# statsleelab/gauss

Measured on AMD Instinct MI355X. Metric: imputed SNPs/sec (whole node) at 1/2/4/8 GPUs; LD-GEMM MFMA TFLOP/s vs peak, higher is better.
Workload: dtype f32

## Files before the change

### gauss_amd/csrc/gauss_job.h

```cpp
#pragma once
#include "gauss_internal.h"
#pragma GCC visibility push(default)
#include "../../include/gauss_hip.h"
#pragma GCC visibility pop

#include <algorithm>
#include <atomic>
#include <chrono>
#include <condition_variable>
#include <cmath>
#include <cstdarg>
#include <cstdio>
#include <cstring>
#include <deque>
#include <functional>
#include <map>
#include <memory>
#include <mutex>
#include <set>
#include <shared_mutex>
#include <thread>
#include <string>
#include <vector>

// ... 258 lines not shown
    char* h_pin = nullptr;
    hipEvent_t begin = nullptr;
    hipEvent_t zeroed = nullptr;
    hipEvent_t done = nullptr;
    struct RunEvents { hipEvent_t gram = nullptr, side = nullptr, pack = nullptr, rows = nullptr, epi = nullptr; };
    RunEvents rev[2];
    Prob* d_probs = nullptr;
    Item* d_items = nullptr;    int n_items = 0;
    int2* d_rowmap = nullptr;   int n_rows = 0;
    std::unique_ptr<Plan> gplan;
    std::vector<int> g0;
    std::vector<std::vector<int2>> win_tiles;
    int2* d_tilemap = nullptr;  int n_tiles = 0;
    int n_tiles_b11 = 0;
    int n_items_b11 = 0;
    bool chain_aside = false;
    int2* d_panelmap = nullptr; int n_panels = 0;
    int2* d_dpanelmap = nullptr; int n_dpanels = 0;
    int2* d_gemmmap = nullptr;  int n_gemm = 0;
    int gemm_ut = 128;
    int2* d_finmap = nullptr;   int n_fin = 0;
    int* d_slctmap = nullptr;   int n_slct = 0;
    int* d_condmap = nullptr;   int n_cond = 0;
    int cond_max_U = 0;
    int* d_csmap = nullptr;     int n_cs = 0;
    int* d_prsmap = nullptr;    int n_prs = 0;
    int prs_max_s = 0, prs_max_M = 0;
    int cs_max_T = 0;
    int* d_susiemap = nullptr;  int n_susie = 0;
    int susie_max_M = 0, susie_max_U = 0, susie_max_T = 0;
    int susie_max_L = 0, susie_max_sweeps = 0, susie_max_nblk = 0;
    int susie_max_k = 0;  bool susie_coloc = false;
    int* d_xsmap = nullptr;     int n_xs = 0;
    int* d_xsleadmap = nullptr; int n_xs_lead = 0;
    int xs_max_M = 0, xs_max_U = 0, xs_max_T = 0, xs_max_L = 0, xs_max_sweeps = 0, xs_max_nblk = 0;
    int2* d_traitsmap = nullptr;  int n_traits = 0;
    int2* d_traitsumap = nullptr; int n_traits_u = 0;
    int2* d_missmap = nullptr;  int n_miss_blk = 0;
    int2* d_misstmap = nullptr; int n_miss_t = 0;
    int2* d_missumap = nullptr; int n_miss_u = 0;
    int2* d_loomap = nullptr;   int n_loo = 0;
    bool needs_fused() const
    { return std::any_of(plans.begin(), plans.end(), [](const Plan& pl) { return pl.rd.needs_fused(); }); }
    int max_nblk = 0;
    int max_npanel = 0;
    int solve_split = 0;
    int own_panel = 0;
    struct StreamGroup { int item0, n_items, row0, n_rows, tile0, n_tiles; };
    std::vector<StreamGroup> sgroups;
    std::vector<hipEvent_t> sevp;
    int max_pop = 1;
    int gram_i8 = 0;
    int gram_packed = 0;
    unsigned long long* d_code3 = nullptr;
    unsigned long long pack_stamp = 0;
    int resample_lds = -1;
    int* d_status = nullptr;
    unsigned long long* d_b11_done = nullptr;
    bool merged = false;
    bool force_merged = false;
    bool queue_touched = false;
    hipStream_t zero_queue = nullptr;
    double wait_bound_us = 0.0;
    unsigned long long merged_runs = 0;
    int n_items_b21_early = 0;
    int n_tiles_b21_early = 0;
    double* d_results = nullptr; size_t n_results = 0;
    double* h_res2[2] = {nullptr, nullptr};
    int* h_st2[2] = {nullptr, nullptr};
    hipEvent_t done2[2] = {nullptr, nullptr};
    unsigned run_seq = 0, fetch_seq = 0;
    double* h_results = nullptr;
    int* h_status = nullptr;
    struct Export { int plan, which; size_t off; int rows, width, pitch; double* user; };
    std::vector<Export> exports;
    std::vector<std::pair<int, int>> exp_chunks;
    std::vector<hipEvent_t> exp_ev;
    double* h_export = nullptr;
    ExportD* d_exports = nullptr;
    bool prof = false;
    std::vector<ProfSlot> slots;
    double prof_ms[5] = {0, 0, 0, 0, 0};
    long long prof_n[5] = {0, 0, 0, 0, 0};
    bool ran = false;
    bool ran_solve = true;
    unsigned prof_run = 0;
    long long n_merged = 0, n_demoted = 0, n_giveups = 0, n_rerun_failed = 0;
};

struct StreamSetup {
    uint8_t* d_m = nullptr;
    uint8_t* d_u = nullptr;
    long long ldraw = 0;
    size_t row_bytes = 0;
    int M = 0, U = 0;
    std::vector<int> first_tile;
    std::vector<int> tile_group;
    std::vector<hipEvent_t> ev;
    std::mutex mu;
    std::condition_variable cv;
    int recorded = 0, rc = 0;
    std::string err;
    int n_groups() const { return (int)first_tile.size() - 1; }
};

struct WinSpec {
// ... 61 lines not shown
```

### gauss_amd/csrc/gauss_plan.cpp

```cpp
#include "gauss_job.h"

static int seg_max_for(const std::vector<WinSpec>& specs)
{
    if (specs.size() >= 4) return 4096;
    double pairs = 0, kp = 0;
    for (const WinSpec& w : specs) {
        if (w.gene_off || w.pair_i || w.M < 1 || w.n_pop < 1 || w.n_pop > 64 || !w.pop_off) return SEG_MAX;
        int nc = 0;
        for (int c = 0; c < 3; c++) nc += (w.u_codings >> c) & 1;
        const double mt = (w.M + TILE - 1) / TILE, ut = ((double)w.U * std::max(nc, 1) + TILE - 1) / TILE;
        pairs += mt * (mt + 1) / 2 + ut * mt;
        kp = std::max(kp, w.draw_pop ? (double)w.n_drawn + 32.0 : (double)w.pop_off[w.n_pop] + 32.0 * w.n_pop);
    }
    const double want = pairs * kp / 1300.0;
    return (int)std::min<double>(SEG_MAX, std::max<double>(384.0, std::floor(want / KC) * KC));
}
static int group_target_for(size_t n_windows)
{
    return n_windows >= 4 ? 2048 : 0;
}
int plan_problem(const WinSpec& w, Plan& pl, int seg_max, int group_target)
{
    if (w.mode != GAUSS_MODE_POOLED && w.mode != GAUSS_MODE_WEIGHTED) return fail(GAUSS_E_INVALID, "bad mode %d", w.mode);
    if (w.n_pop < 1 || w.n_pop > 64) return fail(GAUSS_E_INVALID, "n_pop must be in 1..64 (got %d)", w.n_pop);
    if (!w.pop_off) return fail(GAUSS_E_INVALID, "pop_off is NULL");
    if (w.M < 1) return fail(GAUSS_E_INVALID, "need at least one measured SNP row (got %d)", w.M);
    if (w.U < 0) return fail(GAUSS_E_INVALID, "negative n_unmeasured");
    if (w.mode == GAUSS_MODE_WEIGHTED && !w.pop_wgt) return fail(GAUSS_E_INVALID, "pop_wgt is NULL in weighted mode");
    if (!w.geno_m || (w.U > 0 && !w.geno_u)) return fail(GAUSS_E_INVALID, "genotype pointer is NULL");
    for (int p = 0; p < w.n_pop; p++)
        if (w.pop_off[p + 1] < w.pop_off[p]) return fail(GAUSS_E_INVALID, "pop_off must be non-decreasing");
    if (w.pop_off[0] != 0) return fail(GAUSS_E_INVALID, "pop_off[0] must be 0");
    const int N = w.pop_off[w.n_pop];
    if (N < 1) return fail(GAUSS_E_INVALID, "no samples");
    if ((long long)N * 225 >= (1LL << 31)) return fail(GAUSS_E_RANGE, "%d samples exceed the exact-integer range (9.5 M)", N);
    if (w.geno_fmt != GAUSS_GENO_U8 && w.geno_fmt != GAUSS_GENO_2BIT) return fail(GAUSS_E_INVALID, "bad geno_format %d", w.geno_fmt);
    if (w.geno_fmt == GAUSS_GENO_U8 && w.ld < N) return fail(GAUSS_E_INVALID, "ld (%lld) < n_samples (%d)", w.ld, N);
    if (w.geno_fmt == GAUSS_GENO_2BIT) {
        if (w.ld % 16) return fail(GAUSS_E_INVALID, "2-bit rows need a stride that is a multiple of 16 bytes (got %lld)", w.ld);
        long long end = 0;
        for (int q = 0; q < w.n_pop; q++) {
            const long long blk = (long long)rup((size_t)(w.pop_off[q + 1] - w.pop_off[q]), 64) / 4;
            const long long off = w.pop_src_off ? w.pop_src_off[q] : end;
            if (off < 0 || off % 16) return fail(GAUSS_E_INVALID, "pop_src_off[%d] = %lld is not a multiple of 16", q, off);
            if (off + blk > w.ld) return fail(GAUSS_E_INVALID, "population block %d ends past the row stride", q);
            if (!w.pop_src_off) end = off + blk;
        }
    }
    if (w.kind != GAUSS_WIN_IMPUTE && w.kind != GAUSS_WIN_QCAT && w.kind != GAUSS_WIN_LD)
        return fail(GAUSS_E_INVALID, "bad window kind %d", w.kind);
    if (!w.ld_only && w.kind != GAUSS_WIN_LD && (w.U > 0 || w.kind == GAUSS_WIN_QCAT) && !w.z1) return fail(GAUSS_E_INVALID, "z1 is NULL");
    if (w.u_codings & ~(GAUSS_CODE_ADDITIVE | GAUSS_CODE_DOMINANT | GAUSS_CODE_RECESSIVE))
        return fail(GAUSS_E_INVALID, "bad u_codings mask %d", w.u_codings);
// ... 425 lines not shown
        for (int k = 0; k < K; k++) {
            const int i = mem[(size_t)k];
            const WinSpec& w = specs[(size_t)i];
            Plan::Riders& rd = plans[(size_t)i].rd;
            Prob& p = plans[(size_t)i].p;
            const char* differs = w.susie_L != a.susie_L ? "susie_L" : w.susie_coverage != a.susie_coverage ? "susie_coverage" :
                w.susie_prior_var != a.susie_prior_var ? "susie_prior_var" : w.susie_tol != a.susie_tol ? "susie_tol" :
                w.susie_min_abs_corr != a.susie_min_abs_corr ? "susie_min_abs_corr" : w.susie_max_sweeps != a.susie_max_sweeps ? "susie_max_sweeps" :
                (w.susie_estimate_var != 0) != (a.susie_estimate_var != 0) ? "susie_estimate_var" :
                (w.susie_measured_only != 0) != (a.susie_measured_only != 0) ? "susie_measured_only" : nullptr;
            if (differs) return fail(GAUSS_E_INVALID, "window %d: %s differs from the leader's (window %d): the windows of xs_group = %d share their susie_* arguments", i, differs, lead, id);
            const RiderOuts& o = w.out;
            if (k > 0 && (o.susie_pip || o.susie_set || o.susie_set_pip || o.susie_V || o.susie_lse || o.susie_mass || o.susie_purity || o.susie_size ||
                          o.susie_kept || o.susie_alpha || o.susie_mu || o.susie_sweeps || o.susie_lbf))
                return fail(GAUSS_E_INVALID, "window %d: out_susie_* on a peer of xs_group = %d: the joint fit is returned on the leader (window %d)", i, id, lead);
            if (k > 0 && (o.xs_V || o.xs_purity || o.xs_mu || o.xs_n))
                return fail(GAUSS_E_INVALID, "window %d: out_xs_* on a peer of xs_group = %d: they are the leader's (window %d)", i, id, lead);
            const int T = w.M + w.U;
            if (k > 0 && !w.xs_from_lead && (w.M != a.M || w.U != a.U))
                return fail(GAUSS_E_INVALID, "window %d: xs_from_lead is NULL (the same index) but n_measured / n_unmeasured = %d / %d differ from the leader's %d / %d",
                            i, w.M, w.U, a.M, a.U);
            if (w.xs_from_lead) {
                rd.xs_from_lead.assign(w.xs_from_lead, w.xs_from_lead + TL);
                rd.xs_to_lead.assign((size_t)T, -1);
                for (int j = 0; j < TL; j++) {
                    const int c = rd.xs_from_lead[(size_t)j];
                    if (c < -1 || c >= T)
                        return fail(GAUSS_E_INVALID, "window %d: xs_from_lead[%d] = %d is neither -1 nor a candidate of the window (0 .. %d)", i, j, c, T - 1);
                    if (c >= 0 && rd.xs_to_lead[(size_t)c] >= 0)
                        return fail(GAUSS_E_INVALID, "window %d: xs_from_lead[%d] = xs_from_lead[%d] = %d: two leader candidates cannot be one SNP", i,
                                    rd.xs_to_lead[(size_t)c], j, c);
                    if (c >= 0) rd.xs_to_lead[(size_t)c] = j;
                }
            }
            rd.xs_K = K; rd.xs_pos = k; rd.xs_lead = lead; rd.xs_mu = k == 0 && o.xs_mu != nullptr;
            p.xs_n = K; p.xs_pos = k; p.xs_mu = rd.xs_mu ? 1 : 0;
            for (int s = 0; s < XS_MAX; s++) p.xs_peer[s] = mem[(size_t)std::min(s, K - 1)];
        }
    }
    return GAUSS_OK;
}

int job_build(gauss_ctx* ctx, const std::vector<WinSpec>& specs, int on_device, gauss_job** out, const StreamSetup* stream)
{
    const bool streamed = stream != nullptr;
    const auto tb0 = std::chrono::steady_clock::now();
    gauss_job* job = new gauss_job();
    std::unique_ptr<gauss_job, void (*)(gauss_job*)> guard(job, job_free);
    job->ctx = ctx;
    job->n = (int)specs.size();
    job->on_device = on_device;
    job->gram_i8 = ctx->gram_i8;
    job->gram_packed = (ctx->gram_packed && !ctx->gram_i8) ? 1 : 0;
    job->plans.resize(job->n);
    for (const WinSpec& w : specs)
        if (w.draw_pop && (specs.size() != 1 || streamed)) return fail(GAUSS_E_INVALID, "a resampled window is a job of its own");
    const int seg_max = seg_max_for(specs);
    for (int i = 0; i < job->n; i++) {
        int rc = plan_problem(specs[i], job->plans[i], seg_max, group_target_for(specs.size()));
        if (rc) return rc;
        job->plans[i].p.gram_i8 = job->gram_i8;
        if (!job->plans[i].draw_col.empty()) job->resample_lds = resample_pack_lds_bytes(job->plans[i].p.row_src_bytes);
    }
    {
        const int rc = plan_xs_groups(specs, job->plans);
        if (rc) return rc;
    }
    size_t exp_doubles = 0;
    if (!streamed) {
        for (int i = 0; i < job->n; i++) {
            const Plan& pl = job->plans[i];
            const Prob& p = pl.p;
            const bool has = p.kind == GAUSS_WIN_LD || p.npanel > 0;
            if (!has) continue;
            if (pl.out_b11) { job->exports.push_back(gauss_job::Export{i, 0, exp_doubles, p.M, p.M, p.Mld, pl.out_b11}); exp_doubles += (size_t)p.M * p.M; }
            if (pl.out_b21 && p.U > 0) { job->exports.push_back(gauss_job::Export{i, 1, exp_doubles, p.U, p.M, p.Mld, pl.out_b21}); exp_doubles += (size_t)p.U * p.M; }
            exp_doubles = rup(exp_doubles, 32);
        }
        if (exp_doubles * sizeof(double) > ((size_t)256 << 20)) { job->exports.clear(); exp_doubles = 0; }
    }
    const auto tb1 = std::chrono::steady_clock::now();
    if (on_device && !streamed && job->n >= 2 && env_int("GAUSS_SHARE_MEASURED", 1) != 0) {
        const Plan& a = job->plans[0];
        bool ok = true;
        std::vector<int32_t> gl;
        std::vector<int> g0((size_t)job->n, 0);
        std::set<std::pair<int, int>> have;
        size_t cl0 = 0, own_pairs = 0;
        for (int i = 0; i < job->n && ok; i++) {
            const Plan& b = job->plans[i];
            ok = !b.rows_m.empty() && !b.p.ld_only && !b.p.n_gene && b.p.P <= 32 && b.h_geno_m == a.h_geno_m && b.user_ld == a.user_ld &&
                 b.p.mode == a.p.mode && b.p.P == a.p.P && b.p.geno_fmt == a.p.geno_fmt && b.p.slab16 == a.p.slab16 && b.p.Kp == a.p.Kp &&
                 b.pop_raw_off == a.pop_raw_off && b.pop_pk_off == a.pop_pk_off && b.pop_w == a.pop_w && b.seg_k0 == a.seg_k0 &&
                 b.seg_k1 == a.seg_k1 && b.seg_pop == a.seg_pop && b.run_src == a.run_src && b.run_pk_off == a.run_pk_off &&
                 b.groups == a.groups;
            if (!ok) break;
            const size_t M = b.rows_m.size(), mt = (M + TILE - 1) / TILE;
            own_pairs += mt * (mt + 1) / 2;
            size_t pos = gl.size();
            bool join = false;
            if (gl.size() > cl0 && std::is_sorted(gl.begin() + (ptrdiff_t)cl0, gl.end())) {
                const int32_t first = b.rows_m[0];
                const size_t p0 = (size_t)(std::lower_bound(gl.begin() + (ptrdiff_t)cl0, gl.end(), first) - gl.begin());
                if (p0 < gl.size() && gl[p0] == first) {
                    join = true;
                    for (size_t k = 0; k < M && join; k++) {
// ... 174 lines not shown
            for (int pr = 0; pr < p.npair; pr++) {
                const bool b21 = !p.ld_only && job->plans[i].pair_ti[pr] >= p.Mp / TILE;
                if (shm && !b21) continue;
                (b21 ? tilemap_b21 : tilemap).push_back(make_int2(i, pr));
                job->win_tiles[(size_t)i].push_back(make_int2(i, pr));
            }
        for (int pn = 0; pn < p.npi; pn++) panelmap.push_back(make_int2(i, pn));
        for (int pn = 0; pn < p.npanel; pn++) dpanelmap.push_back(make_int2(i, pn));
        const Plan::Riders& rd = job->plans[i].rd;
        if (rd.loo)
            for (int pn = 0; pn < (p.M + NR - 1) / NR; pn++) loomap.push_back(make_int2(i, pn));
        if (rd.slct_K) slctmap.push_back(i);
        if (rd.cond) { condmap.push_back(i); job->cond_max_U = std::max(job->cond_max_U, p.U); }
        if (rd.cs) { csmap.push_back(i); job->cs_max_T = std::max(job->cs_max_T, p.M + p.U); }
        if (rd.prs_n_s) { prsmap.push_back(i); job->prs_max_s = std::max(job->prs_max_s, rd.prs_n_s); job->prs_max_M = std::max(job->prs_max_M, p.M); }
        if (rd.susie_L && rd.xs_group) {
            xsmap.push_back(i);
            if (rd.xs_pos == 0) xsleadmap.push_back(i);
            job->xs_max_M = std::max(job->xs_max_M, p.M); job->xs_max_T = std::max(job->xs_max_T, p.M + p.U);
            job->xs_max_L = std::max(job->xs_max_L, rd.susie_L); job->xs_max_sweeps = std::max(job->xs_max_sweeps, p.susie_max_sweeps);
            if (!p.susie_measured_only) { job->xs_max_U = std::max(job->xs_max_U, p.U); job->xs_max_nblk = std::max(job->xs_max_nblk, p.nblk); }
        } else if (rd.susie_L) {
            susiemap.push_back(i);
            job->susie_max_M = std::max(job->susie_max_M, p.M); job->susie_max_T = std::max(job->susie_max_T, p.M + p.U);
            job->susie_max_L = std::max(job->susie_max_L, rd.susie_L); job->susie_max_sweeps = std::max(job->susie_max_sweeps, p.susie_max_sweeps);
            job->susie_max_k = std::max(job->susie_max_k, rd.susie_k); job->susie_coloc = job->susie_coloc || rd.coloc;
            if (!p.susie_measured_only) { job->susie_max_U = std::max(job->susie_max_U, p.U); job->susie_max_nblk = std::max(job->susie_max_nblk, p.nblk); }
        }
        if (rd.traits_T) {
            for (int b = 0; b < p.nblk; b++) traitsmap.push_back(make_int2(i, b));
            for (int us = 0; us < (p.U + NB - 1) / NB; us++) traitsumap.push_back(make_int2(i, us));
        }
        if (rd.miss) {
            if (p.miss_nm) for (int b = 0; b < p.nblk; b++) missmap.push_back(make_int2(i, b));
            for (int k = 0; k < p.miss_nm; k++) misstmap.push_back(make_int2(i, k));
            for (int us = 0; us < (p.U + NB - 1) / NB; us++) missumap.push_back(make_int2(i, us));
        }
        if (p.npanel > 0) {
            job->max_nblk = std::max(job->max_nblk, p.nblk); job->max_npanel = std::max(job->max_npanel, p.npi);
            for (int up = 0; up < p.Up128 / job->gemm_ut; up++)
                for (int kb = 0; kb < (p.Mld + 127) / 128; kb++) gemmmap.push_back(make_int2(i, (up << 8) | kb));
            for (int c = 0; c < (p.n_rhs + 255) / 256; c++) finmap.push_back(make_int2(i, c));
        }
        if (p.mode != 0) job->max_pop = std::max(job->max_pop, p.P);
    }
    {
        auto live_rows = [&](const Plan& pl, int t) {
            const Prob& p = pl.p;
            const int mt = p.Mp / TILE;
            if (!pl.tile_live.empty()) return pl.tile_live[(size_t)t];
            const int left = (t < mt) ? p.M - t * TILE : p.U - (t - mt) * TILE;
            return left > TILE ? TILE : left;
        };
        auto halves = [](int r, int w) { const int n = (r - w * 64 + 31) / 32; return n < 0 ? 0 : (n > 2 ? 2 : n); };
        for (ItemH& h : items) {
            h.ord = h.len;
            if (job->gram_i8) continue;
            const Plan& pl = plan_of(h.prob);
            const int ra = live_rows(pl, pl.pair_ti[h.pair]), rb = live_rows(pl, pl.pair_tj[h.pair]);
            const bool packed = job->gram_packed && pl.p.slab16;
            int mx = 0;
            for (int wr = 0; wr < 2; wr++)
                for (int wc = 0; wc < 2; wc++) mx = std::max(mx, (packed ? std::min(halves(ra, wr), 1) : halves(ra, wr)) * halves(rb, wc));
            h.ord = std::max(KC, (h.len * std::max(mx, 1) / 4 + KC - 1) / KC * KC);
        }
    }
    auto is_b11 = [&](const ItemH& h) { return h.b11 != 0; };
    std::vector<uint8_t> item_class(items.size(), 0);
    auto order_items = [&]() {
        int L = 0;
        bool whole = true;
        for (const ItemH& h : items) { L = std::max(L, h.ord / KC); whole = whole && h.ord % KC == 0 && h.ord >= 0; }
        if (!whole || (size_t)L > 4 * items.size() + 1024) {
            std::vector<size_t> idx(items.size());
            for (size_t n = 0; n < idx.size(); n++) idx[n] = n;
            std::stable_sort(idx.begin(), idx.end(), [&](size_t a, size_t b) {
                return item_class[a] != item_class[b] ? item_class[a] < item_class[b] : items[a].ord > items[b].ord; });
            std::vector<ItemH> out(items.size());
            for (size_t n = 0; n < idx.size(); n++) out[n] = items[idx[n]];
            items.swap(out);
            return;
        }
        const size_t nb = (size_t)3 * (size_t)(L + 1);
        std::vector<uint32_t> start(nb + 1, 0u);
        auto bucket = [&](size_t n) { return (size_t)item_class[n] * (size_t)(L + 1) + (size_t)(L - items[n].ord / KC); };
        for (size_t n = 0; n < items.size(); n++) start[bucket(n) + 1]++;
        for (size_t b = 0; b < nb; b++) start[b + 1] += start[b];
        std::vector<ItemH> out(items.size());
        for (size_t n = 0; n < items.size(); n++) out[start[bucket(n)]++] = items[n];
        items.swap(out);
    };
    {
        const int mode = env_int("GAUSS_CHAIN_ASIDE", 1);
        bool genes = false;
        double b21_len = 0.0;
        auto cost_len = [&](const ItemH& h) { return (double)h.len * ((job->gram_packed && plan_of(h.prob).p.slab16) ? GRAM_PACKED_COST : 1.0); };
        for (const ItemH& h : items) if (!is_b11(h)) b21_len += cost_len(h);
        for (int i = 0; i < job->n; i++) genes = genes || job->plans[i].p.n_gene > 0;
        const double t_b21 = b21_len * 2.0 * TILE * TILE / (job->gram_i8 ? 960e12 : 120e12), t_chain = 0.5e-3 + 100e-6 * job->max_nblk;
        {
            double all_len = 0.0;
            for (const ItemH& h : items) all_len += cost_len(h);
            job->wait_bound_us = 50.0 * 1e6 * all_len * 2.0 * TILE * TILE / (job->gram_i8 ? 960e12 : 120e12);
        }
        job->chain_aside = !streamed && mode != 0 && !panelmap.empty() && !tilemap_b21.empty() && !genes && job->ctx->chain &&
                           job->ctx->side && (mode == 2 || t_b21 >= 1.2 * t_chain);
        if (job->chain_aside)
            for (size_t n = 0; n < items.size(); n++) {
                item_class[n] = is_b11(items[n]) ? 0 : 1;
                job->n_items_b11 += is_b11(items[n]) ? 1 : 0;
            }
        {
            const int mm = env_int("GAUSS_CHAIN_MERGED", 1);
            job->merged = job->chain_aside && mm != 0 && (!job->gram_i8 || mm == 2);
            job->force_merged = job->merged && mm == 2;
        }
// ... 384 lines not shown
                return GAUSS_OK;
            };
            int rc = upload(w.raw_m, pl.h_geno_m, pl.rows_m, p.M);
            if (!rc) rc = upload(w.raw_u, pl.h_geno_u, pl.rows_u, pl.U_user);
            if (rc) return rc;
        }
    }
    if (shm) {
        Plan& g = *job->gplan;
        Prob& q = g.p;
        const size_t n = (size_t)job->n;
        char* T = job->d_tab;
        char* W = job->d_ws;
        q.ld_raw = g.user_ld;
        q.raw_m = g.h_geno_m; q.raw_u = nullptr;
        q.packed = (uint8_t*)(W + go.packed); q.packed_u = q.packed;
        q.sx = (int*)(W + go.sx); q.sxx = (int*)(W + go.sxx); q.sx_u = q.sx; q.sxx_u = q.sxx;
        q.rt_sd = (double*)(W + go.sd); q.rt_wm = (double*)(W + go.wm); q.rt_sd_u = q.rt_sd; q.rt_wm_u = q.rt_wm;
        q.rt_mu = (double*)(W + go.mu); q.rt_wmu = (double*)(W + go.wmu); q.rt_mu_u = q.rt_mu; q.rt_wmu_u = q.rt_wmu;
        q.pop_raw_off = (const int*)(T + to[n].raw_off); q.pop_pk_off = (const int*)(T + to[n].pk_off);
        q.pop_w = (const double*)(T + to[n].w); q.pop_wf = (const double*)(T + to[n].wf); q.pop_md = (const double*)(T + to[n].md);
        q.seg_pop = (const int*)(T + to[n].seg_pop); q.seg_k0 = (const int*)(T + to[n].k0); q.seg_k1 = (const int*)(T + to[n].k1);
        q.pop_seg0 = (const int*)(T + to[n].seg0);
        q.pair_ti = (const int*)(T + to[n].ti); q.pair_tj = (const int*)(T + to[n].tj); q.pair_lut = (const int*)(T + to[n].lut);
        q.word_pop = (const uint8_t*)(T + to[n].wp); q.word_run = (const uint8_t*)(T + to[n].wr);
        q.rows_m = (const int*)(T + to[n].rm); q.rows_u = nullptr;
        q.run_pk_off = (const int*)(T + to[n].rpk); q.run_src = (const int*)(T + to[n].rsrc);
        q.slab = (float*)(W + go.slab); q.slab_g = q.slab; q.gpair_ti = q.pair_ti; q.gpair_tj = q.pair_tj; q.g0 = 0; q.n_gpair = q.npair;
        q.z1 = nullptr; q.A = nullptr; q.B21 = nullptr; q.Linv = nullptr; q.V = nullptr; q.Gsum = nullptr; q.Part = nullptr;
        q.out_z = q.out_info = nullptr; clear_riders(q); q.out_ld = nullptr; q.status = job->d_status;
        q.gene_off = nullptr; q.gene_out_off = nullptr; q.n_gene = 0;
        memcpy(blob.data() + o_probs + sizeof(Prob) * n, &q, sizeof(Prob));
    }
    for (size_t n = 0; n < items.size(); n++) {
        const ItemH& h = items[n];
        const Plan& pl = plan_of(h.prob);
        const Prob& p = pl.p;
        const std::pair<int, int>& gr = h.group >= 0 ? pl.groups[h.group] : pl.fine[(size_t)(-1 - h.group)];
        const int ti = pl.pair_ti[h.pair], tj = pl.pair_tj[h.pair];
        const int mt = p.Mp / TILE;
        auto rows = [&](int t) {
            if (!pl.tile_live.empty()) return pl.tile_live[(size_t)t];
            int left = (t < mt) ? p.M - t * TILE : p.U - (t - mt) * TILE; return left > TILE ? TILE : left;
        };
        auto tile_rows = [&](int t) { return t < mt ? p.packed + (size_t)t * TILE * p.Kp : p.packed_u + (size_t)(t - mt) * TILE * p.Kp; };
        Item it;
        it.a = tile_rows(ti);
        it.b = tile_rows(tj);
        it.slab = p.slab + ((size_t)h.pair * p.nseg + gr.first) * (p.slab16 ? TILE * TILE / 2 : TILE * TILE);
        it.seg_k1 = p.seg_k1 + gr.first;
        it.chunk_live = (const uint32_t*)(job->d_tab + to[h.prob].ch);
        it.Kp = p.Kp; it.k0 = pl.seg_k0[gr.first]; it.nseg = gr.second - gr.first;
        it.rows_a = rows(ti); it.rows_b = rows(tj); it.flags = (ti == tj ? 1 : 0) | (p.slab16 ? 2 : 0) | (p.slab16 && job->gram_packed ? 4 : 0);
        if (job->merged && (int)n < job->n_items_b11) it.flags |= 16;
        else if (job->merged && (int)n < job->n_items_b11 + job->n_items_b21_early) it.flags |= 32;
        memcpy(blob.data() + o_items + sizeof(Item) * n, &it, sizeof(Item));
    }
    for (size_t x = 0; x < job->exports.size(); x++) {
        const gauss_job::Export& ex = job->exports[x];
        const Plan& pl = job->plans[(size_t)ex.plan];
        ExportD d;
        d.src = ex.which ? pl.p.B21 : (pl.p.kind == GAUSS_WIN_LD ? pl.p.A : pl.d_b11_copy);
        d.dst = job->h_export + ex.off;
        d.rows = ex.rows; d.width = ex.width; d.pitch = ex.pitch; d.pad_ = 0;
        memcpy(blob.data() + o_exports + sizeof(ExportD) * x, &d, sizeof(ExportD));
    }
    const auto tj2 = std::chrono::steady_clock::now();
    memcpy(job->h_pin, blob.data(), blob.size());
    launch_h2d_copy(job->d_tab, job->h_pin, job->tab_bytes, st);
    HIPCHK(hipGetLastError());
    if (job_trace) {
        auto ms = [](std::chrono::steady_clock::time_point a, std::chrono::steady_clock::time_point b) { return std::chrono::duration<double, std::milli>(b - a).count(); };
        fprintf(stderr, "[job] %d windows: plan %.2f ms (the windows' plans %.2f, shared rows + row checks %.2f, tables + work items %.2f), allocations %.2f ms (workspace %.1f MB, tables %.2f MB, pinned %.2f MB), events + zeroing + tables %.2f ms, table copy queued in %.2f ms\n",
                job->n, ms(tb0, tj0), ms(tb0, tb1), ms(tb1, tb2), ms(tb2, tj0), ms(tj0, tj1), job->ws_bytes / 1e6, job->tab_bytes / 1e6, (pin_tab + 2 * (pin_res + pin_st)) / 1e6, ms(tj1, tj2),
                ms(tj2, std::chrono::steady_clock::now()));
    }
    job->d_probs = (Prob*)(job->d_tab + o_probs);
    job->d_items = (Item*)(job->d_tab + o_items);
    job->d_rowmap = (int2*)(job->d_tab + o_rowmap);
    job->d_tilemap = (int2*)(job->d_tab + o_tilemap);
    job->d_panelmap = (int2*)(job->d_tab + o_panelmap);
    job->d_dpanelmap = (int2*)(job->d_tab + o_dpanelmap);
    job->d_gemmmap = (int2*)(job->d_tab + o_gemmmap);
    job->d_finmap = (int2*)(job->d_tab + o_finmap);
    job->d_loomap = (int2*)(job->d_tab + o_loomap);
    job->d_slctmap = (int*)(job->d_tab + o_slctmap);
    job->d_condmap = (int*)(job->d_tab + o_condmap);
    job->d_csmap = (int*)(job->d_tab + o_csmap);
    job->d_prsmap = (int*)(job->d_tab + o_prsmap);
    job->d_susiemap = (int*)(job->d_tab + o_susiemap);
    job->d_xsmap = (int*)(job->d_tab + o_xsmap);
    job->d_xsleadmap = (int*)(job->d_tab + o_xsleadmap);
    job->d_traitsmap = (int2*)(job->d_tab + o_traitsmap);
    job->d_traitsumap = (int2*)(job->d_tab + o_traitsumap);
    job->d_missmap = (int2*)(job->d_tab + o_missmap);
    job->d_misstmap = (int2*)(job->d_tab + o_misstmap);
    job->d_missumap = (int2*)(job->d_tab + o_missumap);
    job->d_exports = (ExportD*)(job->d_tab + o_exports);
    if (!on_device && !streamed) HIPCHK(hipStreamSynchronize(st));
    std::vector<char>().swap(job->h_tab);
    { std::lock_guard<std::mutex> lock(ctx->mu); ctx->jobs.insert(job); }
    *out = guard.release();
    return GAUSS_OK;
}
```

### gauss_amd/csrc/k_gram.hip

```cpp
#include "gauss_internal.h"
#include "k_gram_common.h"
#include <cstdlib>
#include <type_traits>

#ifndef GAUSS_GRAM_EDGE16
#define GAUSS_GRAM_EDGE16 1
#endif

namespace gauss {

typedef float f32x16 __attribute__((ext_vector_type(16)));
typedef uint32_t u32x4 __attribute__((ext_vector_type(4)));

constexpr int LROW = 64;
constexpr int LTILE = TILE * LROW;

typedef float f32x2 __attribute__((ext_vector_type(2)));

template <int NA, int NB, bool SK10>
__device__ __forceinline__ void chunk_mfma(const uint8_t* __restrict__ la, const uint8_t* __restrict__ lb,
                                           const int (&aoff)[2], const int (&boff)[2], f32x16& acc00, f32x16& acc01,
                                           f32x16& acc10, f32x16& acc11, int nl)
{
#define GAUSS_MFMA_PAIR(AW0, AW1, BW0, BW1, HI)                                                       \
// ... 203 lines not shown
#pragma unroll
        for (int w = 0; w < 4; w++) {
#pragma unroll
            for (int hi = 0; hi < 2; hi++) {
                f32x2 fa = hi ? __builtin_amdgcn_cvt_pk_f32_fp8((int)a[w], true) : __builtin_amdgcn_cvt_pk_f32_fp8((int)a[w], false);
                if (NA > 1) {
                    const f32x2 fa2 = hi ? __builtin_amdgcn_cvt_pk_f32_fp8((int)a2[w], true) : __builtin_amdgcn_cvt_pk_f32_fp8((int)a2[w], false);
                    fa[0] = pk_combine(fa[0], fa2[0]);
                    fa[1] = pk_combine(fa[1], fa2[1]);
                }
#pragma unroll
                for (int nc = 0; nc < NC; nc++) {
                    const f32x2 fb = hi ? __builtin_amdgcn_cvt_pk_f32_fp8((int)b[nc][w], true) : __builtin_amdgcn_cvt_pk_f32_fp8((int)b[nc][w], false);
#pragma unroll
                    for (int e = 0; e < 2; e++) acce[ga][nc] = __builtin_amdgcn_mfma_f32_16x16x4f32(fa[e], fb[e], acce[ga][nc], 0, 0, 0);
                }
            }
            __builtin_amdgcn_sched_barrier(0);
        }
    }
}

template <int NA, int NC, typename OUT>
__device__ __forceinline__ void flush_edge_packed(OUT out, int erow0, int ecol0, const uint32_t (&rune)[2][NC][4])
{
#pragma unroll
    for (int ga = 0; ga < 2; ga++)
#pragma unroll
        for (int nc = 0; nc < NC; nc++) {
            const int o = ((erow0 + 16 * ga) >> 1) * TILE + ecol0 + 16 * nc;
            out[o] = pk_slab_lo(rune[ga][nc][0], rune[ga][nc][1]);
            out[o + TILE] = pk_slab_lo(rune[ga][nc][2], rune[ga][nc][3]);
            if (NA > 1) {
                out[o + 16 * TILE] = pk_slab_hi(rune[ga][nc][0], rune[ga][nc][1]);
                out[o + 17 * TILE] = pk_slab_hi(rune[ga][nc][2], rune[ga][nc][3]);
            }
        }
}

template <int N>
__device__ __forceinline__ void wait_dma_barrier()
{
    asm volatile("s_waitcnt vmcnt(%0) lgkmcnt(0)\n\ts_barrier" ::"n"(N) : "memory");
}
template <int NS>
__device__ __forceinline__ void wait_dma_barrier_dyn(int groups_newer)
{
    if (NS <= 2 || groups_newer <= 0) wait_dma_barrier<0>();
    else if (groups_newer == 1) wait_dma_barrier<4>();
    else wait_dma_barrier<8>();
}

template <int NA, int NB, typename ACC, int NS, bool SK10 = false, int NC = 0, bool PK = false>
__device__ __forceinline__ void run_item(const Item& it, uint8_t* lds, int wr, int wc, int pkf)
{
    const int Kp = it.Kp;
    const auto Ag = it.a;
    const auto Bg = it.b;
    const int tid = threadIdx.x;
    const int lane = tid & 63;
    const int li = lane & 31, lh = lane >> 5;

    const int wave = __builtin_amdgcn_readfirstlane(tid >> 6);
    const int srow = lane >> 2;
    const int spiece = (lane & 3) ^ ((lane >> 4) & 3);
    uint32_t gsrc[2];
#pragma unroll
    for (int j = 0; j < 2; j++) gsrc[j] = (uint32_t)(16 * (wave * 2 + j) + srow) * (uint32_t)Kp + 16u * (uint32_t)spiece;
    typedef __attribute__((address_space(3))) uint8_t* lds_ptr;
    constexpr int RSRC_RAW = 0x00020000;
    const __amdgpu_buffer_rsrc_t rsrc_a = __builtin_amdgcn_make_buffer_rsrc((void*)Ag, 0, TILE * Kp, RSRC_RAW);
    const __amdgpu_buffer_rsrc_t rsrc_b = __builtin_amdgcn_make_buffer_rsrc((void*)Bg, 0, TILE * Kp, RSRC_RAW);

    ACC acc00 = {0}, acc01 = {0}, acc10 = {0}, acc11 = {0};
    uint32_t run0[16], run1[16];
    if (PK) {
#pragma unroll
        for (int r = 0; r < 16; r++) { run0[r] = 0; run1[r] = 0; }
    }

    const int k0 = it.k0;
    const int nseg = it.nseg;
    const auto seg_k1 = it.seg_k1;
    const auto live_tab = it.chunk_live;
    const int klast = uniform_load<int>(seg_k1, nseg - 1);
    auto out = it.slab;
    const int obase = (wr * 64 + 4 * lh) * TILE + wc * 64 + li;
    const int obase16 = (wr * 32 + 2 * lh) * TILE + wc * 64 + li;

#define GAUSS_STAGE(BUF, KOFF)                                                                                   \
    {                                                                                                            \
        _Pragma("unroll") for (int j = 0; j < 2; j++) {                                                        \
            const int t = wave * 2 + j;                                                                          \
            __builtin_amdgcn_raw_ptr_buffer_load_lds(rsrc_a, (lds_ptr)(lds + (BUF) * 2 * LTILE + t * 1024), 16, (int)gsrc[j], (KOFF), 0, 0);          \
            __builtin_amdgcn_raw_ptr_buffer_load_lds(rsrc_b, (lds_ptr)(lds + (BUF) * 2 * LTILE + LTILE + t * 1024), 16, (int)gsrc[j], (KOFF), 0, 0);  \
        }                                                                                                        \
    }
    int cur = 0;
    int kpre = k0;
    int ahead = 0;
#pragma unroll
    for (int d = 0; d < NS - 1; d++)
        if (kpre < klast) { GAUSS_STAGE(d, kpre) kpre += KC; ahead++; }
    wait_dma_barrier_dyn<NS>(ahead - 1);
    ahead--;

    const int sw = (li >> 2) & 3;
    int aoff[2], boff[2];
#pragma unroll
    for (int g = 0; g < 2; g++) {
        aoff[g] = (wr * 64 + li) * LROW + 16 * ((2 * g + lh) ^ sw);
        boff[g] = (wc * 64 + li) * LROW + 16 * ((2 * g + lh) ^ sw);
    }

    constexpr bool BE = NC > 0;
    constexpr int NCE = BE ? NC : 1, NGE = PK ? 2 : 4;
    f32x4 acce[NGE][NCE];
    uint32_t rune[2][NCE][4];
    int eoffa = 0, eoffb = 0, erow0 = 0, ecol0 = 0;
    if (BE) {
        const int r16 = lane & 15, q16 = lane >> 4, sw16 = (r16 >> 2) & 3;
#pragma unroll
        for (int ga = 0; ga < NGE; ga++)
#pragma unroll
            for (int nc = 0; nc < NCE; nc++) {
                acce[ga][nc] = f32x4{0.f, 0.f, 0.f, 0.f};
#pragma unroll
                for (int r = 0; r < 4; r++) if (PK) rune[ga & 1][nc][r] = 0;
            }
        eoffa = (wr * 64 + r16) * LROW + 16 * (q16 ^ sw16);
        eoffb = (wc * 64 + r16) * LROW + 16 * (q16 ^ sw16);
        erow0 = wr * 64 + 4 * q16;
        ecol0 = wc * 64 + r16;
    }

    int k = k0;
    uint32_t lbits = uniform_load<uint32_t>(live_tab, k0 >> 9);
    int nl_next = chunk_live_units(lbits, k0 >> 6);
    for (int seg = 0; seg < nseg; seg++) {
        const int kend = uniform_load<int>(seg_k1, seg);
        int since = 0;
        for (; k < kend; k += KC) {
            if (kpre < klast) {
                int nb_ = cur + NS - 1;
                if (nb_ >= NS) nb_ -= NS;
                GAUSS_STAGE(nb_, kpre)
                kpre += KC;
                ahead++;
            }
            const uint8_t* la = lds + cur * 2 * LTILE;
            const uint8_t* lb = la + LTILE;
            const int nl = nl_next;
            if (k + KC < klast) {
                const int c1 = (k + KC) >> 6;
                if ((c1 & 7) == 0) lbits = uniform_load<uint32_t>(live_tab, c1 >> 3);
                nl_next = chunk_live_units(lbits, c1);
            }
            if constexpr (PK) {
                if (NA > 0 && NB > 0) chunk_mfma_packed<NA, (NB > 0 ? NB : 1)>(la, lb, aoff, boff, acc00, acc01, nl);
                if (BE) chunk_mfma_edge_packed<(NA > 0 ? NA : 1), NCE>(la, lb, eoffa, eoffb, acce);
                if (++since == pkf || k + KC >= kend) {
                    since = 0;
                    if (NA > 0 && NB > 0) {
#pragma unroll
                        for (int r = 0; r < 16; r++) {
                            run0[r] = pk_sub_flush(acc00[r], run0[r]); acc00[r] = 0;
                            if (NB > 1) { run1[r] = pk_sub_flush(acc01[r], run1[r]); acc01[r] = 0; }
                        }
                    }
                    if (BE) {
#pragma unroll
                        for (int ga = 0; ga < 2; ga++)
#pragma unroll
                            for (int nc = 0; nc < NCE; nc++)
#pragma unroll
                                for (int r = 0; r < 4; r++) { rune[ga][nc][r] = pk_sub_flush(acce[ga][nc][r], rune[ga][nc][r]); acce[ga][nc][r] = 0.f; }
                    }
                }
            } else {
                if (NA > 0 && NB > 0) chunk_mfma<NA, (NB > 0 ? NB : 1), SK10>(la, lb, aoff, boff, acc00, acc01, acc10, acc11, nl);
                if (BE) chunk_mfma_edge<(NA > 0 ? NA : 1), NCE>(la, lb, eoffa, eoffb, acce);
            }
            wait_dma_barrier_dyn<NS>(ahead - 1);
            if (ahead > 0) ahead--;
            cur = (cur + 1 == NS) ? 0 : cur + 1;
        }
// ... 3 lines not shown
                int ob = obase16;
                asm volatile("" : "+v"(ob));
#pragma unroll
                for (int r = 0; r < 16; r += 2) {
                    const int o = ob + (((r & 3) + 8 * (r >> 2)) >> 1) * TILE;
                    out[o] = pk_slab_lo(run0[r], run0[r + 1]);
                    if (NB > 1) out[o + 32] = pk_slab_lo(run1[r], run1[r + 1]);
                    if (NA > 1) {
                        out[o + 16 * TILE] = pk_slab_hi(run0[r], run0[r + 1]);
                        if (NB > 1) out[o + 16 * TILE + 32] = pk_slab_hi(run1[r], run1[r + 1]);
                    }
                }
#pragma unroll
                for (int r = 0; r < 16; r++) { run0[r] = 0; run1[r] = 0; }
            }
            if (BE) {
                int er = erow0, ec = ecol0;
                asm volatile("" : "+v"(er), "+v"(ec));
                flush_edge_packed<(NA > 0 ? NA : 1), NCE>(out, er, ec, rune);
#pragma unroll
                for (int ga = 0; ga < 2; ga++)
#pragma unroll
                    for (int nc = 0; nc < NCE; nc++)
#pragma unroll
                        for (int r = 0; r < 4; r++) rune[ga][nc][r] = 0;
            }
            out += TILE * TILE / 2;
        } else {
            if (NA > 0 && NB > 0) {
                int ob = obase, ob16 = obase16;
                asm volatile("" : "+v"(ob), "+v"(ob16));
                flush_acc<NA, (NB > 0 ? NB : 1), SK10>(out, (it.flags & 2) != 0, ob, ob16, acc00, acc01, acc10, acc11);
#pragma unroll
                for (int r = 0; r < 16; r++) { acc00[r] = 0; acc01[r] = 0; acc10[r] = 0; acc11[r] = 0; }
            }
            if (BE) {
                int er = erow0, ec = ecol0;
                asm volatile("" : "+v"(er), "+v"(ec));
                flush_edge<(NA > 0 ? NA : 1), NCE>(out, (it.flags & 2) != 0, er, ec, acce);
#pragma unroll
                for (int ga = 0; ga < 4; ga++)
#pragma unroll
                    for (int nc = 0; nc < NCE; nc++) acce[ga][nc] = f32x4{0.f, 0.f, 0.f, 0.f};
            }
            out += (it.flags & 2) ? TILE * TILE / 2 : TILE * TILE;
        }
    }
}

template <typename ACC, int NS>
__device__ __forceinline__ void gram_item(const Item& it, uint8_t* lds, int pkf)
{
    const int wave = __builtin_amdgcn_readfirstlane(threadIdx.x >> 6);
    const int wr = wave >> 1, wc = wave & 1;

    int na = (it.rows_a - wr * 64 + 31) / 32;
    int nb = (it.rows_b - wc * 64 + 31) / 32;
    na = na < 0 ? 0 : (na > 2 ? 2 : na);
    nb = nb < 0 ? 0 : (nb > 2 ? 2 : nb);
    const bool diag = (it.flags & 1) != 0;
    if (diag && wr == 1 && wc == 0) na = 0;
    int nc = 0;
    if (std::is_same<ACC, f32x16>::value && GAUSS_GRAM_EDGE16 && na > 0) {
        int nb16 = (it.rows_b - wc * 64 + 15) / 16;
        nb16 = nb16 < 0 ? 0 : (nb16 > 4 ? 4 : nb16);
        if (nb16 & 1) nc = nb16;
    }
    if constexpr (std::is_same<ACC, f32x16>::value) {
        if (it.flags & 4) {
            if (nc == 3) { if (na == 2) run_item<2, 0, ACC, NS, false, 3, true>(it, lds, wr, wc, pkf); else run_item<1, 0, ACC, NS, false, 3, true>(it, lds, wr, wc, pkf); }
            else if (nc == 1) { if (na == 2) run_item<2, 0, ACC, NS, false, 1, true>(it, lds, wr, wc, pkf); else run_item<1, 0, ACC, NS, false, 1, true>(it, lds, wr, wc, pkf); }
            else if (na == 0 || nb == 0) run_item<0, 0, ACC, NS>(it, lds, wr, wc, pkf);
            else if (na == 2 && nb == 2) run_item<2, 2, ACC, NS, false, 0, true>(it, lds, wr, wc, pkf);
            else if (na == 2) run_item<2, 1, ACC, NS, false, 0, true>(it, lds, wr, wc, pkf);
            else if (nb == 2) run_item<1, 2, ACC, NS, false, 0, true>(it, lds, wr, wc, pkf);
            else run_item<1, 1, ACC, NS, false, 0, true>(it, lds, wr, wc, pkf);
            return;
        }
    }
    if (nc == 3) { if (na == 2) run_item<2, 0, ACC, NS, false, 3>(it, lds, wr, wc, pkf); else run_item<1, 0, ACC, NS, false, 3>(it, lds, wr, wc, pkf); return; }
    if (nc == 1) { if (na == 2) run_item<2, 0, ACC, NS, false, 1>(it, lds, wr, wc, pkf); else run_item<1, 0, ACC, NS, false, 1>(it, lds, wr, wc, pkf); return; }
    if (na == 0 || nb == 0) run_item<0, 0, ACC, NS>(it, lds, wr, wc, pkf);
    else if (na == 2 && nb == 2 && diag && wr == wc) run_item<2, 2, ACC, NS, true>(it, lds, wr, wc, pkf);
    else if (na == 2 && nb == 2) run_item<2, 2, ACC, NS>(it, lds, wr, wc, pkf);
    else if (na == 2) run_item<2, 1, ACC, NS>(it, lds, wr, wc, pkf);
    else if (nb == 2) run_item<1, 2, ACC, NS>(it, lds, wr, wc, pkf);
    else run_item<1, 1, ACC, NS>(it, lds, wr, wc, pkf);
}

template <typename ACC, int NS, int OCC>
__global__ __launch_bounds__(256, OCC) __attribute__((amdgpu_num_vgpr(52))) void gram_kernel(const Item* __restrict__ items,
                                                                                             unsigned long long* __restrict__ b11_done,
                                                                                             const unsigned long long* __restrict__ code3,
                                                                                             unsigned long long pack_stamp)
{
    __shared__ __attribute__((aligned(16))) uint8_t lds[NS * 2 * LTILE];

    const Item& it = items[blockIdx.x];
    const int counted = it.flags & 48;
    int pkf = PK_F;
    if (code3 && uniform_load<unsigned long long>((GP(const unsigned long long))code3, 0) < pack_stamp) pkf = PK_F_GENO;
    gram_item<ACC, NS>(it, lds, pkf);
    if (counted && b11_done) {
        asm volatile("s_waitcnt vmcnt(0)" ::: "memory");
        __syncthreads();
        if (threadIdx.x == 0) {
            __builtin_amdgcn_fence(__ATOMIC_RELEASE, "agent");
            asm volatile("s_waitcnt vmcnt(0)" ::: "memory");
            __hip_atomic_fetch_add(b11_done + ((counted & 32) ? 8 : 0), 1ull, __ATOMIC_RELAXED, __HIP_MEMORY_SCOPE_AGENT);
        }
    }
}

__global__ __launch_bounds__(64) void wait_count_kernel(const unsigned long long* __restrict__ count, unsigned long long target,
                                                        unsigned long long timeout_ticks, int* __restrict__ status, int n_status)
{
    if (threadIdx.x != 0) return;
    __builtin_amdgcn_s_setprio(3);
    const unsigned long long t0 = wall_clock64();
    for (;;) {
        if (__hip_atomic_load(count, __ATOMIC_RELAXED, __HIP_MEMORY_SCOPE_AGENT) >= target) return;
        if (wall_clock64() - t0 > timeout_ticks) break;
        __builtin_amdgcn_s_sleep(127);
    }
    for (int i = 0; i < n_status; i++) status[i] = 1;
}

__global__ __launch_bounds__(64) void count_up_kernel(unsigned long long* __restrict__ count)
{
    if (threadIdx.x == 0) __hip_atomic_fetch_add(count, 1ull, __ATOMIC_RELEASE, __HIP_MEMORY_SCOPE_AGENT);
}

void launch_count_up(unsigned long long* d_count, hipStream_t s)
{
    hipLaunchKernelGGL(count_up_kernel, dim3(1), dim3(64), 0, s, d_count);
}

void launch_wait_count_for(const unsigned long long* d_count, unsigned long long target, int* d_status, hipStream_t s, double bound_us)
{
    hipLaunchKernelGGL(wait_count_kernel, dim3(1), dim3(64), 0, s, d_count, target, (unsigned long long)(bound_us * 100.0), d_status, 1);
// ... 28 lines not shown
```

### gauss_amd/csrc/k_gram_common.h

```cpp
#pragma once
#include "gauss_internal.h"

namespace gauss {

__device__ __forceinline__ float slab_bits(float v) { return v; }
__device__ __forceinline__ float slab_bits(int v) { return __int_as_float(v); }
__device__ __forceinline__ uint32_t slab_u(float v) { return (uint32_t)v; }
__device__ __forceinline__ uint32_t slab_u(int v) { return (uint32_t)v; }
__device__ __forceinline__ float slab_pair(uint32_t lo, uint32_t hi) { return __uint_as_float((lo & 0xFFFFu) | (hi << 16)); }

template <int NA, int NB, bool SK10, typename OUT, typename ACC>
__device__ __forceinline__ void flush_acc(OUT out, bool slab16, int obase, int obase16, const ACC& acc00, const ACC& acc01,
                                          const ACC& acc10, const ACC& acc11)
{
    if (slab16) {
#pragma unroll
        for (int r = 0; r < 16; r += 2) {
            const int o = obase16 + (((r & 3) + 8 * (r >> 2)) >> 1) * TILE;
            out[o] = slab_pair(slab_u(acc00[r]), slab_u(acc00[r + 1]));
            if (NB > 1) out[o + 32] = slab_pair(slab_u(acc01[r]), slab_u(acc01[r + 1]));
            if (NA > 1) {
                if (!SK10) out[o + 16 * TILE] = slab_pair(slab_u(acc10[r]), slab_u(acc10[r + 1]));
                if (NB > 1) out[o + 16 * TILE + 32] = slab_pair(slab_u(acc11[r]), slab_u(acc11[r + 1]));
            }
        }
    } else {
#pragma unroll
        for (int r = 0; r < 16; r++) {
            const int o = obase + ((r & 3) + 8 * (r >> 2)) * TILE;
            out[o] = slab_bits(acc00[r]);
            if (NB > 1) out[o + 32] = slab_bits(acc01[r]);
            if (NA > 1) {
                if (!SK10) out[o + 32 * TILE] = slab_bits(acc10[r]);
                if (NB > 1) out[o + 32 * TILE + 32] = slab_bits(acc11[r]);
            }
        }
    }
}

}
```

Before: 3.795 million.

## Remap gram kernel waves onto narrow layouts for partially filled tiles

After: 3.866 million, median of 6. +1.9%, better.

```diff
diff --git a/gauss_amd/csrc/gauss_job.h b/gauss_amd/csrc/gauss_job.h
--- a/gauss_amd/csrc/gauss_job.h
+++ b/gauss_amd/csrc/gauss_job.h
@@ -334,6 +334,7 @@
     int max_pop = 1;
     int gram_i8 = 0;
     int gram_packed = 0;
+    int gram_narrow = 0;
     unsigned long long* d_code3 = nullptr;
     unsigned long long pack_stamp = 0;
     int resample_lds = -1;
diff --git a/gauss_amd/csrc/gauss_plan.cpp b/gauss_amd/csrc/gauss_plan.cpp
--- a/gauss_amd/csrc/gauss_plan.cpp
+++ b/gauss_amd/csrc/gauss_plan.cpp
@@ -1,4 +1,5 @@
 #include "gauss_job.h"
+#include "k_gram_common.h"
 
 static int seg_max_for(const std::vector<WinSpec>& specs)
 {
@@ -530,6 +531,7 @@
     job->on_device = on_device;
     job->gram_i8 = ctx->gram_i8;
     job->gram_packed = (ctx->gram_packed && !ctx->gram_i8) ? 1 : 0;
+    job->gram_narrow = (!ctx->gram_i8 && env_int("GAUSS_GRAM_ROTATE", 1) != 0 && env_int("GAUSS_GRAM_NARROW", 1) != 0) ? 1 : 0;
     job->plans.resize(job->n);
     for (const WinSpec& w : specs)
         if (w.draw_pop && (specs.size() != 1 || streamed)) return fail(GAUSS_E_INVALID, "a resampled window is a job of its own");
@@ -810,16 +812,19 @@
             const int left = (t < mt) ? p.M - t * TILE : p.U - (t - mt) * TILE;
             return left > TILE ? TILE : left;
         };
-        auto halves = [](int r, int w) { const int n = (r - w * 64 + 31) / 32; return n < 0 ? 0 : (n > 2 ? 2 : n); };
         for (ItemH& h : items) {
             h.ord = h.len;
             if (job->gram_i8) continue;
             const Plan& pl = plan_of(h.prob);
-            const int ra = live_rows(pl, pl.pair_ti[h.pair]), rb = live_rows(pl, pl.pair_tj[h.pair]);
+            const int ti = pl.pair_ti[h.pair], tj = pl.pair_tj[h.pair];
+            const int ra = live_rows(pl, ti), rb = live_rows(pl, tj);
             const bool packed = job->gram_packed && pl.p.slab16;
+            const int layout = job->gram_narrow ? tile_layout(ra, rb, packed) : LAYOUT_QUAD;
             int mx = 0;
-            for (int wr = 0; wr < 2; wr++)
-                for (int wc = 0; wc < 2; wc++) mx = std::max(mx, (packed ? std::min(halves(ra, wr), 1) : halves(ra, wr)) * halves(rb, wc));
+            for (int w = 0; w < 4; w++) {
+                const WaveWork ww = wave_work(ra, rb, ti == tj, packed, false, w, layout);
+                mx = std::max(mx, (packed ? std::min(ww.na, 1) : ww.na) * ww.nb);
+            }
             h.ord = std::max(KC, (h.len * std::max(mx, 1) / 4 + KC - 1) / KC * KC);
         }
     }
@@ -1310,9 +1315,45 @@
         it.chunk_live = (const uint32_t*)(job->d_tab + to[h.prob].ch);
         it.Kp = p.Kp; it.k0 = pl.seg_k0[gr.first]; it.nseg = gr.second - gr.first;
         it.rows_a = rows(ti); it.rows_b = rows(tj); it.flags = (ti == tj ? 1 : 0) | (p.slab16 ? 2 : 0) | (p.slab16 && job->gram_packed ? 4 : 0);
+        if (job->gram_narrow) it.flags |= tile_layout(it.rows_a, it.rows_b, (it.flags & 4) != 0) << LAYOUT_SHIFT;
         if (job->merged && (int)n < job->n_items_b11) it.flags |= 16;
         else if (job->merged && (int)n < job->n_items_b11 + job->n_items_b21_early) it.flags |= 32;
         memcpy(blob.data() + o_items + sizeof(Item) * n, &it, sizeof(Item));
+    }
+    if (env_int("GAUSS_PLAN_FILL", 0) != 0 && !job->gram_i8) {
+        double mx[2][2] = {{0, 0}, {0, 0}}, mean[2][2] = {{0, 0}, {0, 0}}, full[2] = {0, 0};
+        long n_narrow[2] = {0, 0}, n_uneven[2] = {0, 0}, n_cls[2] = {0, 0};
+        for (size_t n = 0; n < items.size(); n++) {
+            const ItemH& h = items[n];
+            const Plan& pl = plan_of(h.prob);
+            const int ti = pl.pair_ti[h.pair], tj = pl.pair_tj[h.pair];
+            const int mt = pl.p.Mp / TILE;
+            auto rows = [&](int t) {
+                if (!pl.tile_live.empty()) return pl.tile_live[(size_t)t];
+                int left = (t < mt) ? pl.p.M - t * TILE : pl.p.U - (t - mt) * TILE; return left > TILE ? TILE : left;
+            };
+            const int ra = rows(ti), rb = rows(tj), c = h.b11 ? 0 : 1;
+            const bool packed = job->gram_packed && pl.p.slab16;
+            n_cls[c]++;
+            full[c] += h.len;
+            for (int f = 0; f < 2; f++) {
+                const int layout = (f && job->gram_narrow) ? tile_layout(ra, rb, packed) : LAYOUT_QUAD;
+                double m = 0, s = 0;
+                for (int w = 0; w < 4; w++) {
+                    const double l = wave_load(wave_work(ra, rb, ti == tj, packed, true, w, layout), packed);
+                    m = std::max(m, l); s += l;
+                }
+                mx[f][c] += h.len * m; mean[f][c] += h.len * s / 4;
+                if (f && layout != LAYOUT_QUAD) n_narrow[c]++;
+                if (!f && m * 4 > s + 1e-9) n_uneven[c]++;
+            }
+        }
+        for (int c = 0; c < 2; c++) {
+            if (!n_cls[c]) continue;
+            fprintf(stderr, "[fill] %s: %ld items (%ld with unequal waves, %ld narrow), K x tiles %.4e; quadrant roles: max %.4e mean %.4e mean/max %.4f; "
+                            "this job's layouts: max %.4e mean %.4e mean/max %.4f\n", c ? "B21" : "B11", n_cls[c], n_uneven[c], n_narrow[c], full[c],
+                    mx[0][c], mean[0][c], mean[0][c] / mx[0][c], mx[1][c], mean[1][c], mean[1][c] / mx[1][c]);
+        }
     }
     for (size_t x = 0; x < job->exports.size(); x++) {
         const gauss_job::Export& ex = job->exports[x];
diff --git a/gauss_amd/csrc/k_gram.hip b/gauss_amd/csrc/k_gram.hip
--- a/gauss_amd/csrc/k_gram.hip
+++ b/gauss_amd/csrc/k_gram.hip
@@ -279,7 +279,7 @@
 }
 
 template <int NA, int NB, typename ACC, int NS, bool SK10 = false, int NC = 0, bool PK = false>
-__device__ __forceinline__ void run_item(const Item& it, uint8_t* lds, int wr, int wc, int pkf)
+__device__ __forceinline__ void run_item(const Item& it, uint8_t* lds, int r0, int c0, int pkf)
 {
     const int Kp = it.Kp;
     const auto Ag = it.a;
@@ -312,8 +312,8 @@
     const auto live_tab = it.chunk_live;
     const int klast = uniform_load<int>(seg_k1, nseg - 1);
     auto out = it.slab;
-    const int obase = (wr * 64 + 4 * lh) * TILE + wc * 64 + li;
-    const int obase16 = (wr * 32 + 2 * lh) * TILE + wc * 64 + li;
+    const int obase = (r0 + 4 * lh) * TILE + c0 + li;
+    const int obase16 = (r0 / 2 + 2 * lh) * TILE + c0 + li;
 
 #define GAUSS_STAGE(BUF, KOFF)                                                                                   \
     {                                                                                                            \
@@ -336,8 +336,8 @@
     int aoff[2], boff[2];
 #pragma unroll
     for (int g = 0; g < 2; g++) {
-        aoff[g] = (wr * 64 + li) * LROW + 16 * ((2 * g + lh) ^ sw);
-        boff[g] = (wc * 64 + li) * LROW + 16 * ((2 * g + lh) ^ sw);
+        aoff[g] = (r0 + li) * LROW + 16 * ((2 * g + lh) ^ sw);
+        boff[g] = (c0 + li) * LROW + 16 * ((2 * g + lh) ^ sw);
     }
 
     constexpr bool BE = NC > 0;
@@ -355,10 +355,10 @@
 #pragma unroll
                 for (int r = 0; r < 4; r++) if (PK) rune[ga & 1][nc][r] = 0;
             }
-        eoffa = (wr * 64 + r16) * LROW + 16 * (q16 ^ sw16);
-        eoffb = (wc * 64 + r16) * LROW + 16 * (q16 ^ sw16);
-        erow0 = wr * 64 + 4 * q16;
-        ecol0 = wc * 64 + r16;
+        eoffa = (r0 + r16) * LROW + 16 * (q16 ^ sw16);
+        eoffb = (c0 + r16) * LROW + 16 * (q16 ^ sw16);
+        erow0 = r0 + 4 * q16;
+        ecol0 = c0 + r16;
     }
 
     int k = k0;
@@ -468,40 +468,33 @@
 __device__ __forceinline__ void gram_item(const Item& it, uint8_t* lds, int pkf)
 {
     const int wave = __builtin_amdgcn_readfirstlane(threadIdx.x >> 6);
-    const int wr = wave >> 1, wc = wave & 1;
-
-    int na = (it.rows_a - wr * 64 + 31) / 32;
-    int nb = (it.rows_b - wc * 64 + 31) / 32;
-    na = na < 0 ? 0 : (na > 2 ? 2 : na);
-    nb = nb < 0 ? 0 : (nb > 2 ? 2 : nb);
+    constexpr bool F32 = std::is_same<ACC, f32x16>::value;
+    const int layout = (it.flags >> LAYOUT_SHIFT) & 3;
+    const WaveRole ro = wave_role(wave, layout);
+    const int r0 = ro.r0, c0 = ro.c0;
     const bool diag = (it.flags & 1) != 0;
-    if (diag && wr == 1 && wc == 0) na = 0;
-    int nc = 0;
-    if (std::is_same<ACC, f32x16>::value && GAUSS_GRAM_EDGE16 && na > 0) {
-        int nb16 = (it.rows_b - wc * 64 + 15) / 16;
-        nb16 = nb16 < 0 ? 0 : (nb16 > 4 ? 4 : nb16);
-        if (nb16 & 1) nc = nb16;
-    }
+    const WaveWork ww = wave_work(it.rows_a, it.rows_b, diag, F32 && (it.flags & 4) != 0, F32 && GAUSS_GRAM_EDGE16, wave, layout);
+    const int na = ww.na, nb = ww.nb, nc = ww.nc;
     if constexpr (std::is_same<ACC, f32x16>::value) {
         if (it.flags & 4) {
-            if (nc == 3) { if (na == 2) run_item<2, 0, ACC, NS, false, 3, true>(it, lds, wr, wc, pkf); else run_item<1, 0, ACC, NS, false, 3, true>(it, lds, wr, wc, pkf); }
-            else if (nc == 1) { if (na == 2) run_item<2, 0, ACC, NS, false, 1, true>(it, lds, wr, wc, pkf); else run_item<1, 0, ACC, NS, false, 1, true>(it, lds, wr, wc, pkf); }
-            else if (na == 0 || nb == 0) run_item<0, 0, ACC, NS>(it, lds, wr, wc, pkf);
-            else if (na == 2 && nb == 2) run_item<2, 2, ACC, NS, false, 0, true>(it, lds, wr, wc, pkf);
-            else if (na == 2) run_item<2, 1, ACC, NS, false, 0, true>(it, lds, wr, wc, pkf);
-            else if (nb == 2) run_item<1, 2, ACC, NS, false, 0, true>(it, lds, wr, wc, pkf);
-            else run_item<1, 1, ACC, NS, false, 0, true>(it, lds, wr, wc, pkf);
+            if (nc == 3) { if (na == 2) run_item<2, 0, ACC, NS, false, 3, true>(it, lds, r0, c0, pkf); else run_item<1, 0, ACC, NS, false, 3, true>(it, lds, r0, c0, pkf); }
+            else if (nc == 1) { if (na == 2) run_item<2, 0, ACC, NS, false, 1, true>(it, lds, r0, c0, pkf); else run_item<1, 0, ACC, NS, false, 1, true>(it, lds, r0, c0, pkf); }
+            else if (na == 0 || nb == 0) run_item<0, 0, ACC, NS>(it, lds, r0, c0, pkf);
+            else if (na == 2 && nb == 2) run_item<2, 2, ACC, NS, false, 0, true>(it, lds, r0, c0, pkf);
+            else if (na == 2) run_item<2, 1, ACC, NS, false, 0, true>(it, lds, r0, c0, pkf);
+            else if (nb == 2) run_item<1, 2, ACC, NS, false, 0, true>(it, lds, r0, c0, pkf);
+            else run_item<1, 1, ACC, NS, false, 0, true>(it, lds, r0, c0, pkf);
             return;
         }
     }
-    if (nc == 3) { if (na == 2) run_item<2, 0, ACC, NS, false, 3>(it, lds, wr, wc, pkf); else run_item<1, 0, ACC, NS, false, 3>(it, lds, wr, wc, pkf); return; }
-    if (nc == 1) { if (na == 2) run_item<2, 0, ACC, NS, false, 1>(it, lds, wr, wc, pkf); else run_item<1, 0, ACC, NS, false, 1>(it, lds, wr, wc, pkf); return; }
-    if (na == 0 || nb == 0) run_item<0, 0, ACC, NS>(it, lds, wr, wc, pkf);
-    else if (na == 2 && nb == 2 && diag && wr == wc) run_item<2, 2, ACC, NS, true>(it, lds, wr, wc, pkf);
-    else if (na == 2 && nb == 2) run_item<2, 2, ACC, NS>(it, lds, wr, wc, pkf);
-    else if (na == 2) run_item<2, 1, ACC, NS>(it, lds, wr, wc, pkf);
-    else if (nb == 2) run_item<1, 2, ACC, NS>(it, lds, wr, wc, pkf);
-    else run_item<1, 1, ACC, NS>(it, lds, wr, wc, pkf);
+    if (nc == 3) { if (na == 2) run_item<2, 0, ACC, NS, false, 3>(it, lds, r0, c0, pkf); else run_item<1, 0, ACC, NS, false, 3>(it, lds, r0, c0, pkf); return; }
+    if (nc == 1) { if (na == 2) run_item<2, 0, ACC, NS, false, 1>(it, lds, r0, c0, pkf); else run_item<1, 0, ACC, NS, false, 1>(it, lds, r0, c0, pkf); return; }
+    if (na == 0 || nb == 0) run_item<0, 0, ACC, NS>(it, lds, r0, c0, pkf);
+    else if (ww.sk10) run_item<2, 2, ACC, NS, true>(it, lds, r0, c0, pkf);
+    else if (na == 2 && nb == 2) run_item<2, 2, ACC, NS>(it, lds, r0, c0, pkf);
+    else if (na == 2) run_item<2, 1, ACC, NS>(it, lds, r0, c0, pkf);
+    else if (nb == 2) run_item<1, 2, ACC, NS>(it, lds, r0, c0, pkf);
+    else run_item<1, 1, ACC, NS>(it, lds, r0, c0, pkf);
 }
 
 template <typename ACC, int NS, int OCC>
diff --git a/gauss_amd/csrc/k_gram_common.h b/gauss_amd/csrc/k_gram_common.h
--- a/gauss_amd/csrc/k_gram_common.h
+++ b/gauss_amd/csrc/k_gram_common.h
@@ -3,6 +3,58 @@
 
 namespace gauss {
 
+constexpr int LAYOUT_SHIFT = 6;
+constexpr int LAYOUT_QUAD = 0, LAYOUT_NARROW_B = 1, LAYOUT_NARROW_A = 2, LAYOUT_NARROW_AB = 3;
+struct WaveRole { int r0, c0, rows, cols; };
+constexpr WaveRole wave_role(int wave, int layout)
+{
+    return layout == LAYOUT_NARROW_B    ? WaveRole{(wave >> 1) * 64, (wave & 1) * 32, 64, 32}
+           : layout == LAYOUT_NARROW_A  ? WaveRole{0, wave * 32, 64, 32}
+           : layout == LAYOUT_NARROW_AB ? WaveRole{(wave >> 1) * 32, (wave & 1) * 32, 32, 32}
+                                        : WaveRole{(wave >> 1) * 64, (wave & 1) * 64, 64, 64};
+}
+constexpr int tile_layout(int rows_a, int rows_b, bool packed)
+{
+    if (rows_a <= 64 && rows_b <= 64) return packed ? LAYOUT_NARROW_B : LAYOUT_NARROW_AB;
+    return rows_b <= 64 ? LAYOUT_NARROW_B : (rows_a <= 64 ? LAYOUT_NARROW_A : LAYOUT_QUAD);
+}
+
+struct WaveWork { int na, nb, nc; bool sk10; };
+constexpr WaveWork wave_work(int rows_a, int rows_b, bool diag, bool packed, bool edge16, int wave, int layout)
+{
+    const WaveRole ro = wave_role(wave, layout);
+    int na = (rows_a - ro.r0 + 31) / 32, nb = (rows_b - ro.c0 + 31) / 32, nb16 = (rows_b - ro.c0 + 15) / 16;
+    na = na < 0 ? 0 : (na > ro.rows / 32 ? ro.rows / 32 : na);
+    nb = nb < 0 ? 0 : (nb > ro.cols / 32 ? ro.cols / 32 : nb);
+    nb16 = nb16 < 0 ? 0 : (nb16 > ro.cols / 16 ? ro.cols / 16 : nb16);
+    if (diag && ro.r0 >= ro.c0 + ro.cols) na = 0;
+    const int nc = (edge16 && na > 0 && (nb16 & 1)) ? nb16 : 0;
+    return WaveWork{na, nb, nc, diag && !packed && ro.r0 == ro.c0 && na == 2 && nb == 2};
+}
+constexpr double wave_load(const WaveWork& w, bool packed)
+{
+    const int g = w.nc ? w.nc : 2 * w.nb;
+    return packed ? (w.na > 0 ? g / 4.0 : 0.0) : w.na * g / 8.0;
+}
+
+constexpr bool layouts_cover()
+{
+    for (int layout = 0; layout < 4; layout++)
+        for (int r = 0; r < 128; r += 8)
+            for (int c = 0; c < 128; c += 8) {
+                int n = 0;
+                for (int w = 0; w < 4; w++) {
+                    const WaveRole ro = wave_role(w, layout);
+                    n += (r >= ro.r0 && r < ro.r0 + ro.rows && c >= ro.c0 && c < ro.c0 + ro.cols) ? 1 : 0;
+                }
+                const bool in = ((layout & LAYOUT_NARROW_B) ? c < 64 : true) && ((layout & LAYOUT_NARROW_A) ? r < 64 : true);
+                if (n != (in ? 1 : 0)) return false;
+            }
+    return true;
+}
+static_assert(layouts_cover(), "a layout's four blocks tile its live part exactly once");
+
+#if defined(__HIPCC__)
 __device__ __forceinline__ float slab_bits(float v) { return v; }
 __device__ __forceinline__ float slab_bits(int v) { return __int_as_float(v); }
 __device__ __forceinline__ uint32_t slab_u(float v) { return (uint32_t)v; }
@@ -37,5 +89,6 @@
         }
     }
 }
+#endif
 
 }
```
